# sephiroce/srf

Hardware: AMD Instinct MI355X
Metric: acoustic frames/sec through SRF (123-d fbank, 3-iter DR) at 1/2/4/8 MI355X (higher is better)
Workload: dtype fp32; 1 GPU; wsj_c4: SRF L=6 PH=CH=16 DIM=32 LPAD=RPAD=2 DR iter=3, train step (fwd+bwd+allreduce+Adam); utterances_per_gpu=28, frames_per_utterance=800, global_batch=28, parallelism=dp1, launch=hipgraph (fwd+CTC+bwd)

## Files before the change

include/srf.h:

```cpp
#ifndef SRF_H_
#define SRF_H_
#include <stddef.h>

#ifdef __cplusplus
extern "C" {
#endif

int srf_version(void);
const char* srf_last_error(void);

int srf_route_dr_auto_chunks(int B, int T, int N, int din, int lpad, int rpad, int J, int dout);
int srf_route_dr_split_table(int B, int T, int N, int din, int lpad, int rpad, int J, int dout, int n_chunks,
                             int* info, int* table, int capacity);
size_t srf_route_dr_saved_floats(int B, int T, int J, int dout, int iters);
size_t srf_route_dr_fwd_workspace(int B, int T, int N, int din, int lpad, int rpad, int J, int dout, int iters,
                                  int n_chunks);
size_t srf_route_dr_bwd_workspace(int B, int T, int N, int din, int lpad, int rpad, int J, int dout, int iters,
                                  int n_chunks);
int srf_route_dr_fwd(const float* emb, const float* W, const float* bias, int B, int T, int N, int din, int lpad,
                     int rpad, int J, int dout, int iters, int mask_first, int n_chunks, float* v_out,
                     float* saved, void* workspace, size_t workspace_bytes, void* stream);
size_t srf_route_dr_coupling_floats(int B, int T, int N, int din, int lpad, int rpad, int J, int dout, int iters);
int srf_route_dr_fwd_ex(const float* emb, const float* W, const float* bias, int B, int T, int N, int din, int lpad,
                        int rpad, int J, int dout, int iters, int mask_first, int n_chunks, float* v_out,
                        float* saved, float* couplings, void* workspace, size_t workspace_bytes, void* stream);
int srf_route_dr_bwd_ex(const float* emb, const float* W, const float* bias, int B, int T, int N, int din, int lpad,
                        int rpad, int J, int dout, int iters, int mask_first, int n_chunks, const float* saved,
                        const float* couplings, const float* g_v, float* g_emb, float* g_W, float* g_bias,
                        void* workspace, size_t workspace_bytes, void* stream);
int srf_route_dr_bwd_weights_ex(const float* emb, int B, int T, int N, int din, int lpad, int rpad, int J, int dout,
                                int iters, int mask_first, int n_chunks, const float* saved, const float* couplings,
                                float* g_W, float* g_bias, void* workspace, size_t workspace_bytes, void* stream);
int srf_route_dr_bwd_data_ex(const float* emb, const float* W, const float* bias, int B, int T, int N, int din,
                             int lpad, int rpad, int J, int dout, int iters, int mask_first, int n_chunks,
                             const float* saved, const float* couplings, const float* g_v, float* g_emb,
                             void* workspace, size_t workspace_bytes, void* stream);
int srf_set_seed_source(const void* step_counter);
int srf_set_fault_flag(void* flag);
int srf_route_dr_bwd(const float* emb, const float* W, const float* bias, int B, int T, int N, int din, int lpad,
                     int rpad, int J, int dout, int iters, int mask_first, int n_chunks, const float* saved,
                     const float* g_v, float* g_emb, float* g_W, float* g_bias, void* workspace,
                     size_t workspace_bytes, void* stream);
int srf_route_dr_bwd_data(const float* emb, const float* W, const float* bias, int B, int T, int N, int din,
                          int lpad, int rpad, int J, int dout, int iters, int mask_first, int n_chunks,
                          const float* saved, const float* g_v, float* g_emb, void* workspace,
                          size_t workspace_bytes, void* stream);
int srf_route_dr_bwd_weights(const float* emb, int B, int T, int N, int din, int lpad, int rpad, int J, int dout,
                             int iters, int mask_first, int n_chunks, float* g_W, float* g_bias, void* workspace,
                             size_t workspace_bytes, void* stream);

size_t srf_route_sdr_saved_floats(int B, int T, int J, int dout);
size_t srf_route_sdr_fwd_workspace(int B, int T, int N, int din, int lpad, int rpad, int J, int dout);
size_t srf_route_sdr_bwd_workspace(int B, int T, int N, int din, int lpad, int rpad, int J, int dout, int iters);
int srf_route_sdr_fwd(const float* emb, const float* W, const float* bias, int B, int T, int N, int din, int lpad,
                      int rpad, int J, int dout, int iters, int mask_first, float* v_out, float* saved,
                      void* workspace, size_t workspace_bytes, void* stream);
int srf_route_sdr_bwd(const float* emb, const float* W, const float* bias, int B, int T, int N, int din, int lpad,
                      int rpad, int J, int dout, int iters, int mask_first, const float* saved, const float* g_v,
                      float* g_emb, float* g_W, float* g_bias, void* workspace, size_t workspace_bytes,
                      void* stream);

#define SRF_SDR_MAX_ITEMS 8
typedef struct {
  int t0, t1;
  const float* emb;
  const float* W;
  const float* bias;
  const float* WT;
  float* u;
  int v0, vn;
  float* v;
  float* couplings;
  void* workspace;
  size_t workspace_bytes;
  const float* g_v;
// ... 204 lines not shown
```

srf_amd/_lib.py:

```python
import ctypes
import os

_HERE = os.path.dirname(os.path.abspath(__file__))
LIB_PATH = os.environ.get('SRF_LIB_PATH') or os.path.join(_HERE, 'libsrf.so')

_c_int, _c_size, _vp = ctypes.c_int, ctypes.c_size_t, ctypes.c_void_p

SDR_MAX_ITEMS = 8


class SdrRange(ctypes.Structure):
    _fields_ = [('t0', _c_int), ('t1', _c_int), ('emb', _vp), ('W', _vp), ('bias', _vp), ('WT', _vp),
                ('u', _vp), ('v0', _c_int), ('vn', _c_int), ('v', _vp), ('couplings', _vp),
                ('workspace', _vp), ('workspace_bytes', _c_size), ('g_v', _vp), ('carry', _vp),
                ('gu', _vp), ('g0', _c_int), ('gn', _c_int), ('g_emb', _vp), ('g_W', _vp), ('g_bias', _vp),
                ('accumulate', _c_int), ('u_bf16', _c_int), ('group', _c_int), ('gu_factored', _c_int)]


_ranges = ctypes.POINTER(SdrRange)

CAPSNORM_MAX_ITEMS = 8


class CapsnormRange(ctypes.Structure):
    _fields_ = [('t0', _c_int), ('t1', _c_int), ('layer', _c_int), ('x', _vp), ('gamma', _vp), ('beta', _vp),
                ('y', _vp), ('stat', _vp), ('g_y', _vp), ('g_x', _vp), ('gpart', _vp)]


_cn_ranges = ctypes.POINTER(CapsnormRange)

STREAM_ADVANCE_MAX = 32


class StreamBuf(ctypes.Structure):
    _fields_ = [('ptr', _vp), ('row_bytes', _c_size), ('rows_per_stream', _c_int), ('shift', _c_int),
                ('keep', _c_int)]

_SIGNATURES = {
    'srf_version': (_c_int, []),
    'srf_last_error': (ctypes.c_char_p, []),
    'srf_set_seed_source': (_c_int, [_vp]),
    'srf_set_fault_flag': (_c_int, [_vp]),
    'srf_route_dr_auto_chunks': (_c_int, [_c_int] * 8),
    'srf_route_dr_split_table': (_c_int, [_c_int] * 9 + [_vp, _vp, _c_int]),
    'srf_route_dr_saved_floats': (_c_size, [_c_int] * 5),
    'srf_route_dr_fwd_workspace': (_c_size, [_c_int] * 10),
    'srf_route_dr_bwd_workspace': (_c_size, [_c_int] * 10),
    'srf_route_dr_fwd': (_c_int, [_vp, _vp, _vp] + [_c_int] * 11 + [_vp, _vp, _vp, _c_size, _vp]),
    'srf_route_dr_bwd': (_c_int, [_vp, _vp, _vp] + [_c_int] * 11 + [_vp, _vp, _vp, _vp, _vp, _vp, _c_size, _vp]),
    'srf_route_dr_bwd_data': (_c_int, [_vp, _vp, _vp] + [_c_int] * 11 + [_vp, _vp, _vp, _vp, _c_size, _vp]),
    'srf_route_dr_bwd_weights': (_c_int, [_vp] + [_c_int] * 11 + [_vp, _vp, _vp, _c_size, _vp]),
    'srf_route_dr_coupling_floats': (_c_size, [_c_int] * 9),
    'srf_route_dr_fwd_ex': (_c_int, [_vp, _vp, _vp] + [_c_int] * 11 + [_vp, _vp, _vp, _vp, _c_size, _vp]),
    'srf_route_dr_bwd_ex': (_c_int, [_vp, _vp, _vp] + [_c_int] * 11 + [_vp] * 7 + [_c_size, _vp]),
    'srf_route_dr_bwd_data_ex': (_c_int, [_vp, _vp, _vp] + [_c_int] * 11 + [_vp] * 5 + [_c_size, _vp]),
    'srf_route_dr_bwd_weights_ex': (_c_int, [_vp] + [_c_int] * 11 + [_vp] * 5 + [_c_size, _vp]),
    'srf_route_sdr_saved_floats': (_c_size, [_c_int] * 4),
    'srf_route_sdr_fwd_workspace': (_c_size, [_c_int] * 8),
    'srf_route_sdr_bwd_workspace': (_c_size, [_c_int] * 9),
    'srf_route_sdr_fwd': (_c_int, [_vp, _vp, _vp] + [_c_int] * 10 + [_vp, _vp, _vp, _c_size, _vp]),
    'srf_route_sdr_bwd': (_c_int, [_vp, _vp, _vp] + [_c_int] * 10 + [_vp, _vp, _vp, _vp, _vp, _vp, _c_size, _vp]),
    'srf_route_sdr_pose': (_c_int, [_vp, _vp, _vp] + [_c_int] * 10 + [_vp, _c_int, _c_int, _vp]),
    'srf_route_sdr_pose_fp8': (_c_int, [_vp, _vp, _vp] + [_c_int] * 10 + [_vp, _c_int, _c_int, _vp]),
    'srf_route_sdr_recur_workspace': (_c_size, [_c_int] * 5),
    'srf_route_sdr_recur_zero_range': (_c_size, [_c_int] * 5 + [ctypes.POINTER(_c_size)]),
    'srf_route_sdr_coupling_floats': (_c_size, [_c_int] * 4),
    'srf_route_sdr_couplings_required': (_c_int, [_c_int] * 4),
    'srf_route_sdr_fact_floats': (_c_size, [_c_int] * 4),
    'srf_route_sdr_recur_fwd': (_c_int, [_vp] + [_c_int] * 11 + [_vp, _vp, _vp, _c_size, _vp]),
    'srf_route_sdr_recur_bwd': (_c_int, [_vp, _c_int, _c_int, _vp, _vp, _vp] + [_c_int] * 9
                                + [_vp, _vp, _c_int, _c_int, _vp, _c_size, _vp]),
    'srf_route_sdr_transpose_w': (_c_int, [_vp] + [_c_int] * 4 + [_vp, _vp]),
    'srf_route_sdr_gx': (_c_int, [_vp, _c_int, _c_int, _vp] + [_c_int] * 10 + [_vp, _vp]),
    'srf_route_sdr_gw': (_c_int, [_vp, _c_int, _c_int, _vp] + [_c_int] * 11 + [_vp, _vp, _vp]),
    'srf_route_sdr_pose_n': (_c_int, [_ranges] + [_c_int] * 10 + [_vp]),
    'srf_route_sdr_recur_fwd_n': (_c_int, [_ranges] + [_c_int] * 8 + [_vp]),
    'srf_route_sdr_recur_bwd_n': (_c_int, [_ranges] + [_c_int] * 8 + [_vp]),
    'srf_route_sdr_gx_n': (_c_int, [_ranges] + [_c_int] * 9 + [_vp]),
    'srf_route_sdr_gw_n': (_c_int, [_ranges] + [_c_int] * 9 + [_vp]),
    'srf_route_sdr_gx_gw_n': (_c_int, [_ranges] + [_c_int] * 9 + [_vp]),
    'srf_route_sdr_gx_gw_fact_n': (_c_int, [_ranges] + [_c_int] * 10 + [_vp]),
    'srf_cnnfe_out_dims': (_c_int, [_c_int, _c_int, ctypes.POINTER(_c_int), ctypes.POINTER(_c_int)]),
    'srf_cnnfe_saved_bytes': (_c_size, [_c_int] * 4),
    'srf_cnnfe_fwd_workspace': (_c_size, [_c_int] * 4),
    'srf_cnnfe_bwd_workspace': (_c_size, [_c_int] * 4),
    'srf_cnnfe_fwd': (_c_int, [_vp, _vp] + [_c_int] * 4 + [_vp] * 16 + [_c_int, ctypes.c_float, ctypes.c_ulonglong,
                                                                       _vp, _vp, _c_size, _vp, _c_size, _vp]),
    'srf_cnnfe_bwd': (_c_int, [_vp, _vp] + [_c_int] * 4 + [_vp] * 4 + [ctypes.c_float, ctypes.c_ulonglong]
                      + [_vp] * 15 + [_c_size, _vp]),
    'srf_cnnfe_bwd_parts': (_c_int, [_c_int, _vp, _vp] + [_c_int] * 4 + [_vp] * 4 + [ctypes.c_float, ctypes.c_ulonglong]
                            + [_vp] * 15 + [_c_size, _vp]),
    'srf_primary_caps_saved_bytes': (_c_size, [_c_int] * 4),
    'srf_primary_caps_bwd_workspace': (_c_size, [_c_int] * 5),
    'srf_primary_caps_fwd': (_c_int, [_vp, _vp] + [_c_int] * 5 + [_vp] * 8 + [_c_int, ctypes.c_float, ctypes.c_float,
                                                                           ctypes.c_ulonglong, _vp, _vp, _c_size, _vp]),
    'srf_primary_caps_bwd': (_c_int, [_vp, _vp] + [_c_int] * 5 + [_vp] * 5 + [_c_int, ctypes.c_float, ctypes.c_float,
                                                                           ctypes.c_ulonglong] + [_vp] * 12
                             + [_c_size, _vp]),
    'srf_primary_caps_fwd_ex': (_c_int, [_vp, _vp] + [_c_int] * 5 + [_vp] * 8
                                + [_c_int, ctypes.c_float, ctypes.c_float, ctypes.c_ulonglong, ctypes.c_float, _c_int,
                                   _vp, _vp, _c_size, _vp]),
    'srf_primary_caps_bwd_ex': (_c_int, [_vp, _vp] + [_c_int] * 5 + [_vp] * 5
                                + [_c_int, ctypes.c_float, ctypes.c_float, ctypes.c_ulonglong, ctypes.c_float]
                                + [_vp] * 12 + [_c_size, _vp]),
    'srf_capsnorm_bwd_workspace': (_c_size, [_c_int] * 3),
# ... 87 lines not shown
```

srf_amd/csrc/route_dr.hip:

```cpp
#include <algorithm>
#include <cmath>
#include <type_traits>

#include "srf_common.h"
#include "route_fwd32.h"
#include "../../include/srf.h"
#include "../../include/srf_prof.h"

namespace {

constexpr float kSquashEps = 1e-7f;

thread_local hipEvent_t* t_ev_start = nullptr;
thread_local hipEvent_t* t_ev_stop = nullptr;
thread_local int t_ev_n = 0;
constexpr int MODE_FWD = 0;
constexpr int MODE_BWD = 1;

using srf::DrGeom;

template <int KS>
__device__ __forceinline__ void load_vec(const float* __restrict__ p, float (&v)[KS]) {
  if constexpr (KS % 4 == 0) {
#pragma unroll
// ... 2356 lines not shown
  const bool bal = p.bal_G > 0;
  const int n_wg = bal ? p.bal_G : p.n_ftiles * p.n_chunks;
  info[0] = bal ? 1 : 0;
  info[1] = n_wg;
  info[2] = p.n_ftiles * in_n;
  info[3] = p.n_slots;
  info[4] = p.plan_arg;
  int n = 0;
  auto emit = [&](int w, int ft, int i0, int i1, int slot) {
    if (n < capacity) {
      int* row = table + (size_t)n * 5;
      row[0] = w, row[1] = ft, row[2] = i0, row[3] = i1, row[4] = slot;
    }
    ++n;
  };
  for (int w = 0; w < n_wg; ++w) {
    if (!bal) {
      const int ft = w / p.n_chunks, slot = w - ft * p.n_chunks;
      const int i0 = slot * p.chunk_len;
      emit(w, ft, std::min(i0, in_n), std::min(in_n, i0 + p.chunk_len), slot);
      continue;
    }
    int u = srf::bal_first(w, p.bal_U, p.bal_G);
    const int u1 = srf::bal_first(w + 1, p.bal_U, p.bal_G);
    while (u < u1) {
      const int ft = u / in_n, i0 = u - ft * in_n, i1 = std::min(in_n, i0 + (u1 - u));
      emit(w, ft, i0, i1, w - srf::bal_owner(ft * in_n, p.bal_U, p.bal_G));
      u += i1 - i0;
    }
  }
  return n;
}

size_t srf_route_dr_saved_floats(int B, int T, int J, int dout, int iters) {
  return (size_t)2 * iters * B * T * J * dout;
}

size_t srf_route_dr_fwd_workspace(int B, int T, int N, int din, int lpad, int rpad, int J, int dout, int iters,
                                  int n_chunks) {
  (void)iters;
  return query(B, T, N, din, lpad, rpad, J, dout, 1, n_chunks).fwd_bytes;
}

size_t srf_route_dr_bwd_workspace(int B, int T, int N, int din, int lpad, int rpad, int J, int dout, int iters,
                                  int n_chunks) {
  return query(B, T, N, din, lpad, rpad, J, dout, iters, n_chunks).ws.bytes;
}

size_t srf_route_dr_coupling_floats(int B, int T, int N, int din, int lpad, int rpad, int J, int dout, int iters) {
  const DrPlan p = query(B, T, N, din, lpad, rpad, J, dout, iters, 0);
  return p.can_store ? p.cpl.total : 0;
}

int srf_route_dr_fwd(const float* emb, const float* W, const float* bias, int B, int T, int N, int din, int lpad,
                     int rpad, int J, int dout, int iters, int mask_first, int n_chunks, float* v_out, float* saved,
                     void* workspace, size_t workspace_bytes, void* stream) {
  return srf_route_dr_fwd_ex(emb, W, bias, B, T, N, din, lpad, rpad, J, dout, iters, mask_first, n_chunks, v_out,
                             saved, nullptr, workspace, workspace_bytes, stream);
}

int srf_route_dr_fwd_ex(const float* emb, const float* W, const float* bias, int B, int T, int N, int din, int lpad,
                        int rpad, int J, int dout, int iters, int mask_first, int n_chunks, float* v_out,
                        float* saved, float* couplings, void* workspace, size_t workspace_bytes, void* stream) {
  DrPlan p;
  const int rc = enter(p, DrGeom{B, T, N, din, lpad, rpad, J, dout, iters, mask_first ? 1 : 0}, n_chunks,
                       emb && W && bias && v_out && saved && workspace, couplings != nullptr, true, workspace_bytes);
  if (rc) return rc;
  return dispatch_din(din, [&](auto D) {
    return fwd_impl<D>(p, emb, W, bias, v_out, saved, couplings, static_cast<float*>(workspace),
                       static_cast<hipStream_t>(stream));
  });
}

int srf_route_dr_bwd(const float* emb, const float* W, const float* bias, int B, int T, int N, int din, int lpad,
                     int rpad, int J, int dout, int iters, int mask_first, int n_chunks, const float* saved,
                     const float* g_v, float* g_emb, float* g_W, float* g_bias, void* workspace,
                     size_t workspace_bytes, void* stream) {
  return route_dr_bwd_entry(emb, W, bias, B, T, N, din, lpad, rpad, J, dout, iters, mask_first, n_chunks, saved,
                            nullptr, g_v, g_emb, g_W, g_bias, workspace, workspace_bytes, stream, true);
}

int srf_route_dr_bwd_ex(const float* emb, const float* W, const float* bias, int B, int T, int N, int din, int lpad,
                        int rpad, int J, int dout, int iters, int mask_first, int n_chunks, const float* saved,
                        const float* couplings, const float* g_v, float* g_emb, float* g_W, float* g_bias,
                        void* workspace, size_t workspace_bytes, void* stream) {
  return route_dr_bwd_entry(emb, W, bias, B, T, N, din, lpad, rpad, J, dout, iters, mask_first, n_chunks, saved,
                            couplings, g_v, g_emb, g_W, g_bias, workspace, workspace_bytes, stream, true);
}

int srf_route_dr_bwd_data(const float* emb, const float* W, const float* bias, int B, int T, int N, int din,
                          int lpad, int rpad, int J, int dout, int iters, int mask_first, int n_chunks,
                          const float* saved, const float* g_v, float* g_emb, void* workspace,
                          size_t workspace_bytes, void* stream) {
  return srf_route_dr_bwd_data_ex(emb, W, bias, B, T, N, din, lpad, rpad, J, dout, iters, mask_first, n_chunks, saved,
                                  nullptr, g_v, g_emb, workspace, workspace_bytes, stream);
}

int srf_route_dr_bwd_data_ex(const float* emb, const float* W, const float* bias, int B, int T, int N, int din,
                             int lpad, int rpad, int J, int dout, int iters, int mask_first, int n_chunks,
                             const float* saved, const float* couplings, const float* g_v, float* g_emb,
                             void* workspace, size_t workspace_bytes, void* stream) {
  float* unused = reinterpret_cast<float*>(workspace);
  return route_dr_bwd_entry(emb, W, bias, B, T, N, din, lpad, rpad, J, dout, iters, mask_first, n_chunks, saved,
                            couplings, g_v, g_emb, unused, unused, workspace, workspace_bytes, stream, false);
}

// ... 23 lines not shown
```

srf_amd/csrc/route_fwd32.hip:

```cpp
#include <cmath>
#include <cstdint>
#include <cstdlib>
#include <algorithm>
#include <type_traits>

#include "srf_common.h"
#include "route_fwd32.h"


#ifndef SRF_DR_IL
#define SRF_DR_IL 1
#endif

#ifndef SRF_DR_BAL_AUTO
#define SRF_DR_BAL_AUTO 1
#endif

namespace {

typedef __bf16 bf8 __attribute__((ext_vector_type(8)));
typedef __bf16 bf4 __attribute__((ext_vector_type(4)));
typedef _Float16 h8 __attribute__((ext_vector_type(8)));
typedef float f16v __attribute__((ext_vector_type(16)));

__device__ __forceinline__ f16v mfma32(const bf8& a, const bf8& b, const f16v& c) {
  return __builtin_amdgcn_mfma_f32_32x32x16_bf16(a, b, c, 0, 0, 0);
}
__device__ __forceinline__ f16v mfma32h(const h8& a, const h8& b, const f16v& c) {
  return __builtin_amdgcn_mfma_f32_32x32x16_f16(a, b, c, 0, 0, 0);
}

__device__ __forceinline__ float exp2i(int e) { return srf_exp2i(e); }
__device__ __forceinline__ int split_exp(float m) { return srf_split_exp(m); }

__device__ __forceinline__ void split3(float a, __bf16& a1, __bf16& a2, __bf16& a3) {
  a1 = (__bf16)a;
  const float r = a - (float)a1;
  a2 = (__bf16)r;
  a3 = (__bf16)(r - (float)a2);
}

__device__ __forceinline__ void split2h(float a, _Float16& a1, _Float16& a2) { srf_split2h(a, a1, a2); }

__device__ __forceinline__ void split8h(const float* __restrict__ src, bool ok, float s, _Float16* d1,
                                        _Float16* d2) {
  f4 lo = {0.f, 0.f, 0.f, 0.f}, hi = lo;
  if (ok) {
    lo = *reinterpret_cast<const f4*>(src);
    hi = *reinterpret_cast<const f4*>(src + 4);
  }
  const float v[8] = {lo.x, lo.y, lo.z, lo.w, hi.x, hi.y, hi.z, hi.w};
  h8 p1, p2;
#pragma unroll
  for (int k = 0; k < 8; ++k) {
    _Float16 a1, a2;
    split2h(v[k] * s, a1, a2);
    p1[k] = a1;
    p2[k] = a2;
  }
  *reinterpret_cast<h8*>(d1) = p1;
  *reinterpret_cast<h8*>(d2) = p2;
}

constexpr int kAbsBlocks = 128;
__global__ __launch_bounds__(256) void absmax_kernel(const float* __restrict__ a, size_t na,
                                                     const float* __restrict__ b, size_t nb, float* part) {
  const float* p = blockIdx.y ? b : a;
  const size_t n = blockIdx.y ? nb : na;
  float m = 0.f;
  const size_t stride = (size_t)gridDim.x * blockDim.x;
  size_t i = (size_t)blockIdx.x * blockDim.x + threadIdx.x;
  if ((reinterpret_cast<uintptr_t>(p) & 15) == 0) {
    const size_t n4 = n / 4;
    for (; i < n4; i += stride) {
      const f4 v = reinterpret_cast<const f4*>(p)[i];
      m = fmaxf(m, fmaxf(fmaxf(fabsf(v.x), fabsf(v.y)), fmaxf(fabsf(v.z), fabsf(v.w))));
    }
    i = n4 * 4 + (size_t)blockIdx.x * blockDim.x + threadIdx.x;
  }
  for (; i < n; i += stride) m = fmaxf(m, fabsf(p[i]));
#pragma unroll
  for (int o = 32; o >= 1; o >>= 1) m = fmaxf(m, __shfl_xor(m, o, 64));
  __shared__ float wm[4];
  if ((threadIdx.x & 63) == 0) wm[threadIdx.x >> 6] = m;
  __syncthreads();
  if (threadIdx.x == 0) part[blockIdx.y * kAbsBlocks + blockIdx.x] = fmaxf(fmaxf(wm[0], wm[1]), fmaxf(wm[2], wm[3]));
}

struct PrepArgs {
  const float *W, *bias, *emb;
  _Float16 *Ws, *xs;
  __bf16* bs;
  float *bsum, *WT, *xT;
  const float* part;
  float* hdr;
  int in_n, JD, JDp, din, n_chunks, chunk_len, F, N, T, lpad, Fp;
  int wt16;
  int xt16;
  size_t xplane;
  size_t n_a, n_b, n_c, n_d, n_e;
  size_t n_f, xt_block0;
};

constexpr int kXtTile = 64;

__global__ __launch_bounds__(256) void prep32_kernel(PrepArgs P) {
  if (P.n_f && blockIdx.x >= P.xt_block0) {
    __shared__ float tile[kXtTile][32 + 1];
    __shared__ int sbx;
    const int ntile = (P.Fp + kXtTile - 1) / kXtTile;
    const int blk = blockIdx.x - (int)P.xt_block0;
    const int i = blk / ntile, f0 = (blk - i * ntile) * kXtTile;
    const int w = i / P.N, n = i - w * P.N;
    if (P.xt16 && threadIdx.x < 64) {
      float m = 0.f;
      for (int k = threadIdx.x; k < kAbsBlocks; k += 64) m = fmaxf(m, P.part[kAbsBlocks + k]);
#pragma unroll
      for (int o = 32; o >= 1; o >>= 1) m = fmaxf(m, __shfl_xor(m, o, 64));
      if (threadIdx.x == 0) sbx = split_exp(m);
    }
    for (int k = threadIdx.x; k < kXtTile * P.din; k += blockDim.x) {
      const int fl = k / P.din, e = k - fl * P.din;
      const int f = f0 + fl;
      float v = 0.f;
      if (f < P.F) {
        const int b = f / P.T, t = f - b * P.T;
        const int ts = t + w - P.lpad;
        if (ts >= 0 && ts < P.T) v = P.emb[((size_t)(b * P.T + ts) * P.N + n) * P.din + e];
      }
      tile[fl][e] = v;
    }
    __syncthreads();
    if (P.xt16) {
      const float sc = exp2i(sbx);
      _Float16* x16 = reinterpret_cast<_Float16*>(P.xT);
      for (int k = threadIdx.x; k < (kXtTile / 16) * 32 * 2; k += blockDim.x) {
        const int hf = k & 1, e = (k >> 1) & 31, kb = k >> 6;
        const int fb = f0 + kb * 16;
        if (fb >= P.Fp) continue;
        h8 p1, p2;
#pragma unroll
        for (int q = 0; q < 8; ++q) {
          _Float16 a1, a2;
          split2h(tile[kb * 16 + hf * 8 + q][e] * sc, a1, a2);
          p1[q] = a1;
          p2[q] = a2;
        }
        const size_t base = (((size_t)i * (P.Fp / 16) + fb / 16) * 2 * 32 + e) * 16 + hf * 8;
        *reinterpret_cast<h8*>(x16 + base) = p1;
        *reinterpret_cast<h8*>(x16 + base + 32 * 16) = p2;
      }
      return;
    }
    for (int k = threadIdx.x; k < kXtTile * P.din; k += blockDim.x) {
      const int e = k / kXtTile, fl = k - e * kXtTile;
      const int f = f0 + fl;
      if (f < P.Fp) P.xT[((size_t)i * P.din + e) * P.Fp + f] = tile[fl][e];
    }
    return;
  }
  __shared__ int sexp[2];
  const size_t b0 = (size_t)blockIdx.x * blockDim.x, b1 = b0 + blockDim.x;
  const size_t ec = P.n_a + P.n_b, sd = ec + P.n_c, ed = sd + P.n_d;
  const bool split_work = b0 < ec || (b1 > sd && b0 < ed) || (P.wt16 && b1 > ed && b0 < ed + P.n_e);
  if (split_work && threadIdx.x < 128) {
    const int y = threadIdx.x >> 6, l = threadIdx.x & 63;
    float m = 0.f;
    for (int k = l; k < kAbsBlocks; k += 64) m = fmaxf(m, P.part[y * kAbsBlocks + k]);
#pragma unroll
    for (int o = 32; o >= 1; o >>= 1) m = fmaxf(m, __shfl_xor(m, o, 64));
    if (l == 0) sexp[y] = split_exp(m);
  }
  if (split_work) __syncthreads();
  const int aw = split_work ? sexp[0] : 0, bx = split_work ? sexp[1] : 0;
  if (blockIdx.x == 0 && threadIdx.x == 0) {
    P.hdr[0] = exp2i(-(aw + bx));
    P.hdr[1] = (float)aw;
    P.hdr[2] = (float)bx;
  }
  size_t idx = (size_t)blockIdx.x * blockDim.x + threadIdx.x;
  if (idx < P.n_a) {
    const size_t e0 = idx * 8;
    const int e = e0 % P.din;
    const size_t rr = e0 / P.din;
    const int row = rr % P.JDp;
    const size_t i = rr / P.JDp;
    const size_t nw = (size_t)P.in_n * P.JDp * P.din;
    split8h(P.W + (i * P.JD + min(row, P.JD - 1)) * P.din + e, row < P.JD, exp2i(aw), P.Ws + e0, P.Ws + nw + e0);
    return;
  }
  idx -= P.n_a;
  if (idx < P.n_b) {
    const int row = idx % P.JDp;
    const size_t i = idx / P.JDp;
    const float b = row < P.JD ? P.bias[i * P.JD + row] * exp2i(aw + bx) : 0.f;
    __bf16 b1, b2, b3;
    split3(b, b1, b2, b3);
    bf4 v = {b1, b2, b3, (__bf16)0.f};
    *reinterpret_cast<bf4*>(P.bs + idx * 4) = v;
    return;
  }
  idx -= P.n_b;
  if (idx < P.n_c) {
    const int c = idx / P.JD, row = idx - (size_t)c * P.JD;
    const int i0 = c * P.chunk_len, i1 = min(P.in_n, i0 + P.chunk_len);
    float acc = 0.f;
    for (int i = i0; i < i1; i += 8) {
      float v[8];
#pragma unroll
      for (int k = 0; k < 8; ++k) v[k] = i + k < i1 ? P.bias[(size_t)(i + k) * P.JD + row] : 0.f;
#pragma unroll
      for (int k = 0; k < 8; ++k) acc += v[k];
    }
    P.bsum[idx] = acc;
    return;
  }
  idx -= P.n_c;
  if (idx < P.n_d) {
    const size_t e0 = idx * 8;
    const size_t n_data = (size_t)P.F * P.N * P.din;
    const int e = e0 % P.din;
    const size_t rr = e0 / P.din;
    const int f = rr % P.F;
    const int n = rr / P.F;
    const bool ok = e0 < n_data;
    split8h(P.emb + ((size_t)(ok ? f : 0) * P.N + (ok ? n : 0)) * P.din + (ok ? e : 0), ok, exp2i(bx), P.xs + e0,
            P.xs + P.xplane + e0);
    return;
  }
  idx -= P.n_d;
  if (P.wt16 && idx < P.n_e) {
    const int e = idx % P.din;
    const size_t r1 = idx / P.din;
    const int h = r1 % 2;
    const size_t r2 = r1 / 2;
    const int nt16 = (P.JD + 15) / 16;
    const int t = r2 % nt16;
    const size_t i = r2 / nt16;
    const int row = t * 16 + 8 * h;
    const float* w = P.W + (i * P.JD + min(row, P.JD - 1)) * P.din + e;
    const float s = exp2i(aw);
    h8 p1, p2;
#pragma unroll
    for (int k = 0; k < 8; ++k) {
      _Float16 a1, a2;
      split2h(row + k < P.JD ? w[(size_t)k * P.din] * s : 0.f, a1, a2);
      p1[k] = a1;
      p2[k] = a2;
    }
    _Float16* d = reinterpret_cast<_Float16*>(P.WT);
    *reinterpret_cast<h8*>(d + idx * 8) = p1;
    *reinterpret_cast<h8*>(d + P.n_e * 8 + idx * 8) = p2;
    return;
  }
  if (idx < P.n_e) {
    const int e = idx % P.din;
    const size_t r1 = idx / P.din;
    const int g = r1 % 4;
    const size_t r2 = r1 / 4;
    const int nt16 = (P.JD + 15) / 16;
    const int t = r2 % nt16;
    const size_t i = r2 / nt16;
    const int row = t * 16 + 4 * g;
    const float* w = P.W + (i * P.JD + min(row, P.JD - 1)) * P.din + e;
    f4 v;
#pragma unroll
    for (int q = 0; q < 4; ++q) v[q] = row + q < P.JD ? w[(size_t)q * P.din] : 0.f;
// ... 1680 lines not shown
      best = c;
    }
  }
  p.n_chunks = best;
  p.chunk_len = (in_n + best - 1) / best;
  p.bal_G = 0;
  p.bal_U = 0;
  p.n_slots = best;
  p.plan_arg = best;
  {
    const long long U = (long long)n_ftiles * in_n;
    long long G = force_bal ? (n_chunks & (kBalFlag - 1)) : 0;
    if (G <= 0) G = slots;
    G = std::min(G, U);
    const bool fits = U * (G + 1) < (1ll << 31);
    if (fits && forced <= 0) {
      const int len = (int)((U + G - 1) / G);
      const int segs = (len - 1 + in_n - 1) / in_n + 1;
      int n_slots = 1;
      for (int ft = 0; ft < n_ftiles; ++ft) n_slots = std::max(n_slots, bal_tile_slots(ft, in_n, (int)U, (int)G));
      const double cost = (double)(len + kSegCost * segs) * (1.0 + 0.002 * n_slots);
      if (force_bal || (SRF_DR_BAL_AUTO && din == 32 && p.NW > 1 && p.TW == 2 && cost < best_cost)) {
        p.bal_G = (int)G;
        p.bal_U = (int)U;
        p.n_slots = n_slots;
        p.plan_arg = kBalFlag | (int)G;
      }
    }
  }
  p.ws_bsum = srf::align_up((size_t)best * JD * 4, 256);
  p.ws_slab = srf::align_up((size_t)std::max(best, p.n_slots) * F * JD * 4, 256);
  return p;
}

const float* fwd32_hdr(const Fwd32Shape& p, const void* planes) {
  return reinterpret_cast<const float*>(static_cast<const char*>(planes) + p.ws_w + p.ws_b + p.ws_x);
}
size_t fwd32_planes_bytes(const Fwd32Shape& p) { return p.ws_w + p.ws_b + p.ws_x + p.ws_h; }
size_t fwd32_scratch_bytes(const Fwd32Split& p) { return p.ws_bsum + p.ws_slab; }
size_t fwd32_workspace(const Fwd32Plan& p) { return fwd32_planes_bytes(p) + fwd32_scratch_bytes(p); }
float* fwd32_slab(const Fwd32Split& p, void* scratch) {
  return reinterpret_cast<float*>(static_cast<char*>(scratch) + p.ws_bsum);
}

size_t fwd32_lds(const Fwd32Shape& p) {
  return (size_t)p.NW * p.TW * 4 * 64 * 16 + (p.NW > 1 ? (size_t)2 * 32 * p.NW * 8 : 0);
}

int fwd32_prepare(const Fwd32Plan& p, const DrGeom& g, const float* emb, const float* W, const float* bias,
                  void* planes, void* scratch, float* WT, float* xT, hipStream_t st, bool wt16, bool xt16) {
  char* base = static_cast<char*>(planes);
  float* hdr = reinterpret_cast<float*>(base + p.ws_w + p.ws_b + p.ws_x);
  const int din = g.din;
  hipLaunchKernelGGL(absmax_kernel, dim3(kAbsBlocks, 2), dim3(256), 0, st, W, (size_t)g.in_n() * g.JD() * din, emb,
                     (size_t)g.F() * g.N * din, hdr + 64);
  SRF_LAUNCH_CHECK("absmax");
  PrepArgs P;
  P.W = W;
  P.bias = bias;
  P.emb = emb;
  P.Ws = reinterpret_cast<_Float16*>(base);
  P.bs = reinterpret_cast<__bf16*>(base + p.ws_w);
  P.xs = reinterpret_cast<_Float16*>(base + p.ws_w + p.ws_b);
  P.part = hdr + 64;
  P.hdr = hdr;
  P.bsum = reinterpret_cast<float*>(scratch);
  P.WT = WT;
  P.xT = xT;
  P.T = g.T;
  P.lpad = g.lpad;
  P.Fp = (g.F() + 15) / 16 * 16;
  P.in_n = g.in_n();
  P.JD = g.JD();
  P.JDp = p.JDp;
  P.din = din;
  P.n_chunks = p.n_chunks;
  P.chunk_len = p.chunk_len;
  P.F = g.F();
  P.N = g.N;
  P.xplane = p.xplane;
  P.n_a = (size_t)P.in_n * p.JDp * din / 8;
  P.n_b = (size_t)P.in_n * p.JDp;
  P.n_c = (size_t)p.n_chunks * P.JD;
  P.n_d = p.xplane / 8;
  SRF_REQUIRE(!wt16 || din == 32, "prep32: split W^T planes need din 32, got %d", din);
  P.wt16 = wt16 ? 1 : 0;
  SRF_REQUIRE(!xt16 || din == 32, "prep32: split x^T planes need din 32, got %d", din);
  P.xt16 = xt16 ? 1 : 0;
  P.n_e = WT ? (size_t)P.in_n * ((P.JD + 15) / 16) * (wt16 ? 2 : 4) * din : 0;
  SRF_REQUIRE(din <= 32, "prep32: xT tile holds din <= 32, got %d", din);
  P.n_f = xT ? (size_t)P.in_n * ((P.Fp + kXtTile - 1) / kXtTile) : 0;
  P.xt_block0 = (P.n_a + P.n_b + P.n_c + P.n_d + P.n_e + 255) / 256;
  hipLaunchKernelGGL(prep32_kernel, dim3(P.xt_block0 + P.n_f), dim3(256), 0, st, P);
  SRF_LAUNCH_CHECK("prep32");
  return SRF_OK;
}

template <int V>
using Int = std::integral_constant<int, V>;

template <class Fn>
static int dispatch_row(const DrGeom& g, const char* what, Fn&& fn) {
  if (g.din == g.dout) {
    switch (g.din) {
      case 8: return fn(Int<8>{}, Int<8>{});
      case 16: return fn(Int<16>{}, Int<16>{});
      case 32: return fn(Int<32>{}, Int<32>{});
    }
  }
  srf::set_error("%s: unsupported din %d dout %d", what, g.din, g.dout);
  return SRF_EUNSUPPORTED;
}

template <int DIN, class Fn>
static int dispatch_tiles(const Fwd32Shape& p, Fn&& fn) {
  if (p.TW == 2) {
    if constexpr (DIN <= 16) {
      return p.NW == 1 ? fn(Int<1>{}, Int<2>{}) : fn(Int<2>{}, Int<2>{});
    } else {
      switch (p.NW) {
        case 1: return fn(Int<1>{}, Int<2>{});
        case 2: return fn(Int<2>{}, Int<2>{});
        case 4: return fn(Int<4>{}, Int<2>{});
        default: return fn(Int<8>{}, Int<2>{});
      }
    }
  }
  switch (p.NW) {
    case 1: return fn(Int<1>{}, Int<kTW>{});
    case 2: return fn(Int<2>{}, Int<kTW>{});
    case 4: return fn(Int<4>{}, Int<kTW>{});
    default: return fn(Int<kMaxNW>{}, Int<kTW>{});
  }
}

template <int NW, int TW, class Kern, class... Args>
static int launch_rpass(const Fwd32Plan& p, const char* name, Kern piped, Kern plain, hipStream_t st,
                        const Args&... args) {
  const size_t lds = fwd32_lds(p);
  const Kern kern = (NW > 1 && TW <= 2) ? piped : plain;
  if (lds > 64 * 1024)
    SRF_HIP_TRY(hipFuncSetAttribute((const void*)kern, hipFuncAttributeMaxDynamicSharedMemorySize, (int)lds));
// ... 142 lines not shown
```

Baseline: 3.011 million frames/s.

## Add one-pass prep32 kernel that reads each input once via LDS tiles

```diff
diff --git a/include/srf.h b/include/srf.h
--- a/include/srf.h
+++ b/include/srf.h
@@ -21,6 +21,9 @@
                      int rpad, int J, int dout, int iters, int mask_first, int n_chunks, float* v_out,
                      float* saved, void* workspace, size_t workspace_bytes, void* stream);
 size_t srf_route_dr_coupling_floats(int B, int T, int N, int din, int lpad, int rpad, int J, int dout, int iters);
+#define SRF_DR_LAYOUT_N 17
+int srf_route_dr_operand_layout(int B, int T, int N, int din, int lpad, int rpad, int J, int dout, int iters,
+                                long long* out);
 int srf_route_dr_fwd_ex(const float* emb, const float* W, const float* bias, int B, int T, int N, int din, int lpad,
                         int rpad, int J, int dout, int iters, int mask_first, int n_chunks, float* v_out,
                         float* saved, float* couplings, void* workspace, size_t workspace_bytes, void* stream);
diff --git a/srf_amd/_lib.py b/srf_amd/_lib.py
--- a/srf_amd/_lib.py
+++ b/srf_amd/_lib.py
@@ -51,6 +51,7 @@
     'srf_route_dr_bwd_data': (_c_int, [_vp, _vp, _vp] + [_c_int] * 11 + [_vp, _vp, _vp, _vp, _c_size, _vp]),
     'srf_route_dr_bwd_weights': (_c_int, [_vp] + [_c_int] * 11 + [_vp, _vp, _vp, _c_size, _vp]),
     'srf_route_dr_coupling_floats': (_c_size, [_c_int] * 9),
+    'srf_route_dr_operand_layout': (_c_int, [_c_int] * 9 + [_vp]),
     'srf_route_dr_fwd_ex': (_c_int, [_vp, _vp, _vp] + [_c_int] * 11 + [_vp, _vp, _vp, _vp, _c_size, _vp]),
     'srf_route_dr_bwd_ex': (_c_int, [_vp, _vp, _vp] + [_c_int] * 11 + [_vp] * 7 + [_c_size, _vp]),
     'srf_route_dr_bwd_data_ex': (_c_int, [_vp, _vp, _vp] + [_c_int] * 11 + [_vp] * 5 + [_c_size, _vp]),
diff --git a/srf_amd/csrc/route_dr.hip b/srf_amd/csrc/route_dr.hip
--- a/srf_amd/csrc/route_dr.hip
+++ b/srf_amd/csrc/route_dr.hip
@@ -2432,6 +2432,41 @@
   return p.can_store ? p.cpl.total : 0;
 }
 
+int srf_route_dr_operand_layout(int B, int T, int N, int din, int lpad, int rpad, int J, int dout, int iters,
+                                long long* out) {
+  SRF_REQUIRE(out != nullptr, "operand_layout: null argument");
+  DrPlan p;
+  const DrGeom g{B, T, N, din, lpad, rpad, J, dout, iters, 0};
+  if (const int rc = check_geom(g)) return rc;
+  resolve(p, g, 0, true);
+  if (!p.couplings) {
+    srf::set_error("operand_layout: no coupling storage for this shape");
+    return SRF_EUNSUPPORTED;
+  }
+  const srf::Fwd32Shape& s = p.p32;
+  const size_t in_n = g.in_n(), Fp = padded_frames(g);
+  const size_t pl = p.cpl.planes;
+  const size_t v[SRF_DR_LAYOUT_N] = {pl,
+                                     2 * in_n * s.JDp * g.din * 2,
+                                     pl + s.ws_w / 4,
+                                     in_n * s.JDp * 8,
+                                     pl + (s.ws_w + s.ws_b) / 4,
+                                     2 * s.xplane * 2,
+                                     pl + (s.ws_w + s.ws_b + s.ws_x) / 4,
+                                     3 * sizeof(float),
+                                     p.cpl.WT,
+                                     in_n * g.din * ((size_t)g.NT() * 16) * 4,
+                                     p.cpl.xT,
+                                     in_n * g.din * Fp * 4,
+                                     (size_t)s.JDp,
+                                     s.xplane,
+                                     Fp,
+                                     p.gx == GxPass::kStored16 ? 1u : 0u,
+                                     p.gw == GwPass::kGw16s ? 1u : 0u};
+  for (int k = 0; k < SRF_DR_LAYOUT_N; ++k) out[k] = (long long)v[k];
+  return SRF_OK;
+}
+
 int srf_route_dr_fwd(const float* emb, const float* W, const float* bias, int B, int T, int N, int din, int lpad,
                      int rpad, int J, int dout, int iters, int mask_first, int n_chunks, float* v_out, float* saved,
                      void* workspace, size_t workspace_bytes, void* stream) {
diff --git a/srf_amd/csrc/route_fwd32.hip b/srf_amd/csrc/route_fwd32.hip
--- a/srf_amd/csrc/route_fwd32.hip
+++ b/srf_amd/csrc/route_fwd32.hip
@@ -14,6 +14,10 @@
 
 #ifndef SRF_DR_BAL_AUTO
 #define SRF_DR_BAL_AUTO 1
+#endif
+
+#ifndef SRF_PREP32_ONEPASS
+#define SRF_PREP32_ONEPASS 1
 #endif
 
 namespace {
@@ -63,8 +67,12 @@
 }
 
 constexpr int kAbsBlocks = 128;
-__global__ __launch_bounds__(256) void absmax_kernel(const float* __restrict__ a, size_t na,
-                                                     const float* __restrict__ b, size_t nb, float* part) {
+constexpr int kAbsThreads = SRF_PREP32_ONEPASS ? 1024 : 256;
+__device__ __forceinline__ float absmax4(const f4& v) {
+  return fmaxf(fmaxf(fabsf(v.x), fabsf(v.y)), fmaxf(fabsf(v.z), fabsf(v.w)));
+}
+__global__ __launch_bounds__(kAbsThreads) void absmax_kernel(const float* __restrict__ a, size_t na,
+                                                             const float* __restrict__ b, size_t nb, float* part) {
   const float* p = blockIdx.y ? b : a;
   const size_t n = blockIdx.y ? nb : na;
   float m = 0.f;
@@ -72,6 +80,13 @@
   size_t i = (size_t)blockIdx.x * blockDim.x + threadIdx.x;
   if ((reinterpret_cast<uintptr_t>(p) & 15) == 0) {
     const size_t n4 = n / 4;
+    if (SRF_PREP32_ONEPASS) {
+      for (; i + 3 * stride < n4; i += 4 * stride) {
+        const f4* q = reinterpret_cast<const f4*>(p) + i;
+        const f4 v0 = q[0], v1 = q[stride], v2 = q[2 * stride], v3 = q[3 * stride];
+        m = fmaxf(m, fmaxf(fmaxf(absmax4(v0), absmax4(v1)), fmaxf(absmax4(v2), absmax4(v3))));
+      }
+    }
     for (; i < n4; i += stride) {
       const f4 v = reinterpret_cast<const f4*>(p)[i];
       m = fmaxf(m, fmaxf(fmaxf(fabsf(v.x), fabsf(v.y)), fmaxf(fabsf(v.z), fabsf(v.w))));
@@ -81,10 +96,14 @@
   for (; i < n; i += stride) m = fmaxf(m, fabsf(p[i]));
 #pragma unroll
   for (int o = 32; o >= 1; o >>= 1) m = fmaxf(m, __shfl_xor(m, o, 64));
-  __shared__ float wm[4];
+  __shared__ float wm[kAbsThreads / 64];
   if ((threadIdx.x & 63) == 0) wm[threadIdx.x >> 6] = m;
   __syncthreads();
-  if (threadIdx.x == 0) part[blockIdx.y * kAbsBlocks + blockIdx.x] = fmaxf(fmaxf(wm[0], wm[1]), fmaxf(wm[2], wm[3]));
+  if (threadIdx.x == 0) {
+#pragma unroll
+    for (int k = 1; k < kAbsThreads / 64; ++k) m = fmaxf(m, wm[k]);
+    part[blockIdx.y * kAbsBlocks + blockIdx.x] = m;
+  }
 }
 
 struct PrepArgs {
@@ -100,9 +119,206 @@
   size_t xplane;
   size_t n_a, n_b, n_c, n_d, n_e;
   size_t n_f, xt_block0;
+  int rpad, n_xblk, n_wblk, w_bpc;
 };
 
 constexpr int kXtTile = 64;
+
+__device__ __forceinline__ void prep_bs(const PrepArgs& P, size_t idx, int aw, int bx) {
+  const int row = idx % P.JDp;
+  const size_t i = idx / P.JDp;
+  const float b = row < P.JD ? P.bias[i * P.JD + row] * exp2i(aw + bx) : 0.f;
+  __bf16 b1, b2, b3;
+  split3(b, b1, b2, b3);
+  bf4 v = {b1, b2, b3, (__bf16)0.f};
+  *reinterpret_cast<bf4*>(P.bs + idx * 4) = v;
+}
+
+__device__ __forceinline__ void prep_bsum(const PrepArgs& P, size_t idx) {
+  const int c = idx / P.JD, row = idx - (size_t)c * P.JD;
+  const int i0 = c * P.chunk_len, i1 = min(P.in_n, i0 + P.chunk_len);
+  float acc = 0.f;
+  for (int i = i0; i < i1; i += 8) {
+    float v[8];
+#pragma unroll
+    for (int k = 0; k < 8; ++k) v[k] = i + k < i1 ? P.bias[(size_t)(i + k) * P.JD + row] : 0.f;
+#pragma unroll
+    for (int k = 0; k < 8; ++k) acc += v[k];
+  }
+  P.bsum[idx] = acc;
+}
+
+constexpr int kXHaloMax = 16;
+constexpr int kXImgStride = kXtTile + kXHaloMax + 1;
+
+__device__ __forceinline__ int wave_split_exp(const float* __restrict__ part, int y) {
+  const int l = threadIdx.x & 63;
+  float m = fmaxf(part[y * kAbsBlocks + l], part[y * kAbsBlocks + 64 + l]);
+  static_assert(kAbsBlocks == 128, "two block maxima per lane");
+#pragma unroll
+  for (int o = 32; o >= 1; o >>= 1) m = fmaxf(m, __shfl_xor(m, o, 64));
+  return split_exp(m);
+}
+
+__device__ __forceinline__ void split4w(const f4& v, float s, uint32_t (&w)[4]) {
+#pragma unroll
+  for (int j = 0; j < 4; ++j) {
+    _Float16 a1, a2;
+    split2h(v[j] * s, a1, a2);
+    w[j] = (uint32_t)__builtin_bit_cast(uint16_t, a1) | ((uint32_t)__builtin_bit_cast(uint16_t, a2) << 16);
+  }
+}
+__device__ __forceinline__ uint32_t pack_hi(uint32_t a, uint32_t b) { return (a & 0xffffu) | (b << 16); }
+__device__ __forceinline__ uint32_t pack_lo(uint32_t a, uint32_t b) { return (a >> 16) | (b & 0xffff0000u); }
+
+typedef uint32_t u2v __attribute__((ext_vector_type(2)));
+typedef uint32_t u4v __attribute__((ext_vector_type(4)));
+
+constexpr int kWTileStride = 36;
+constexpr int kPrepLdsWords = 4 * 64 * kWTileStride;
+static_assert(32 * kXImgStride + kXtTile <= kPrepLdsWords && (32 * kXImgStride) % 4 == 0, "x image + tt fit");
+
+__device__ __forceinline__ void prep_x_tile(const PrepArgs& P, int blk, uint32_t* lds) {
+  uint32_t* const img = lds;
+  int* const tt = reinterpret_cast<int*>(lds + 32 * kXImgStride);
+  const int tid = threadIdx.x;
+  const int tile = blk / P.N, n = blk - tile * P.N;
+  const int f0 = tile * kXtTile;
+  const int nrow = kXtTile + P.lpad + P.rpad;
+  constexpr int kIt = (kXtTile + kXHaloMax) * 8 / 256 + ((kXtTile + kXHaloMax) * 8 % 256 ? 1 : 0);
+  f4 v[kIt];
+#pragma unroll
+  for (int it = 0; it < kIt; ++it) {
+    const int k = tid + it * 256, r = k >> 3, e4 = k & 7;
+    const int fr = f0 - P.lpad + r;
+    v[it] = f4{0.f, 0.f, 0.f, 0.f};
+    if (r < nrow && fr >= 0 && fr < P.F)
+      v[it] = *reinterpret_cast<const f4*>(P.emb + ((size_t)fr * P.N + n) * 32 + 4 * e4);
+  }
+  if (tid < kXtTile) {
+    const int f = f0 + tid;
+    tt[tid] = f < P.F ? f - (f / P.T) * P.T : -(1 << 24);
+  }
+  if (blk == 0 && tid < 8) {
+    const h8 z = {};
+    *reinterpret_cast<h8*>(P.xs + (size_t)(tid >> 2) * P.xplane + (P.xplane - 32) + (tid & 3) * 8) = z;
+  }
+  const float sc = exp2i(wave_split_exp(P.part, 1));
+#pragma unroll
+  for (int it = 0; it < kIt; ++it) {
+    const int k = tid + it * 256, r = k >> 3, e4 = k & 7;
+    const int fr = f0 - P.lpad + r;
+    if (r >= nrow) continue;
+    uint32_t w[4];
+    split4w(v[it], sc, w);
+    if (P.xT) {
+#pragma unroll
+      for (int j = 0; j < 4; ++j) img[(4 * e4 + j) * kXImgStride + r] = w[j];
+    }
+    if (r >= P.lpad && r < P.lpad + kXtTile && fr < P.F) {
+      _Float16* d = P.xs + ((size_t)n * P.F + fr) * 32 + 4 * e4;
+      *reinterpret_cast<u2v*>(d) = u2v{pack_hi(w[0], w[1]), pack_hi(w[2], w[3])};
+      *reinterpret_cast<u2v*>(d + P.xplane) = u2v{pack_lo(w[0], w[1]), pack_lo(w[2], w[3])};
+    }
+  }
+  if (!P.xT) return;
+  __syncthreads();
+  const int e = tid & 31, hf = (tid >> 5) & 1, kb = tid >> 6;
+  const int fb = f0 + kb * 16;
+  if (fb >= P.Fp) return;
+  int t8[8];
+  {
+    const u4v a = *reinterpret_cast<const u4v*>(&tt[kb * 16 + hf * 8]);
+    const u4v b = *reinterpret_cast<const u4v*>(&tt[kb * 16 + hf * 8 + 4]);
+#pragma unroll
+    for (int q = 0; q < 4; ++q) t8[q] = (int)a[q] - P.lpad, t8[4 + q] = (int)b[q] - P.lpad;
+  }
+  _Float16* x16 = reinterpret_cast<_Float16*>(P.xT);
+  const uint32_t* col = img + e * kXImgStride + kb * 16 + hf * 8;
+  const int nwin = P.lpad + P.rpad + 1;
+  for (int w = 0; w < nwin; ++w) {
+    uint32_t c[8];
+#pragma unroll
+    for (int q = 0; q < 8; ++q) c[q] = (uint32_t)(t8[q] + w) < (uint32_t)P.T ? col[w + q] : 0u;
+    const size_t i = (size_t)w * P.N + n;
+    const size_t base = ((i * (P.Fp / 16) + fb / 16) * 2 * 32 + e) * 16 + hf * 8;
+    *reinterpret_cast<u4v*>(x16 + base) =
+        u4v{pack_hi(c[0], c[1]), pack_hi(c[2], c[3]), pack_hi(c[4], c[5]), pack_hi(c[6], c[7])};
+    *reinterpret_cast<u4v*>(x16 + base + 32 * 16) =
+        u4v{pack_lo(c[0], c[1]), pack_lo(c[2], c[3]), pack_lo(c[4], c[5]), pack_lo(c[6], c[7])};
+  }
+}
+
+__device__ __forceinline__ void prep_w_rows(const PrepArgs& P, int blk, uint32_t* lds) {
+  const int i = blk / P.w_bpc, rb = blk - i * P.w_bpc;
+  const int lane = threadIdx.x & 63, wv = threadIdx.x >> 6;
+  const int e4 = lane & 7, g = lane >> 3;
+  const int rw0 = rb * 256 + wv * 64;
+  const bool active = rw0 < P.JDp;
+  uint32_t* const t = lds + wv * 64 * kWTileStride;
+  f4 v[8];
+#pragma unroll
+  for (int k = 0; k < 8; ++k) {
+    const int row = rw0 + g * 8 + k;
+    v[k] = f4{0.f, 0.f, 0.f, 0.f};
+    if (row < P.JD) v[k] = *reinterpret_cast<const f4*>(P.W + ((size_t)i * P.JD + row) * 32 + 4 * e4);
+  }
+  const float s = exp2i(wave_split_exp(P.part, 0));
+#pragma unroll
+  for (int k = 0; k < 8; ++k) {
+    uint32_t w[4];
+    split4w(v[k], s, w);
+    *reinterpret_cast<u4v*>(t + (g * 8 + k) * kWTileStride + 4 * e4) = u4v{w[0], w[1], w[2], w[3]};
+  }
+  __syncthreads();
+  if (!active) return;
+  const size_t nw = (size_t)P.in_n * P.JDp * 32;
+#pragma unroll
+  for (int it = 0; it < 4; ++it) {
+    const int rl = it * 16 + (lane >> 2), c8 = (lane & 3) * 8;
+    const u4v a = *reinterpret_cast<const u4v*>(t + rl * kWTileStride + c8);
+    const u4v b = *reinterpret_cast<const u4v*>(t + rl * kWTileStride + c8 + 4);
+    _Float16* d = P.Ws + ((size_t)i * P.JDp + rw0 + rl) * 32 + c8;
+    *reinterpret_cast<u4v*>(d) = u4v{pack_hi(a[0], a[1]), pack_hi(a[2], a[3]), pack_hi(b[0], b[1]), pack_hi(b[2], b[3])};
+    *reinterpret_cast<u4v*>(d + nw) =
+        u4v{pack_lo(a[0], a[1]), pack_lo(a[2], a[3]), pack_lo(b[0], b[1]), pack_lo(b[2], b[3])};
+  }
+  if (P.WT == nullptr) return;
+  const int nt16 = (P.JD + 15) / 16;
+  const int e = lane & 31;
+#pragma unroll
+  for (int it = 0; it < 4; ++it) {
+    const int g2 = it * 2 + (lane >> 5);
+    const int r0 = rw0 + g2 * 8;
+    if (r0 >= nt16 * 16) continue;
+    uint32_t c[8];
+#pragma unroll
+    for (int q = 0; q < 8; ++q) c[q] = t[(g2 * 8 + q) * kWTileStride + e];
+    _Float16* d = reinterpret_cast<_Float16*>(P.WT) + (((size_t)i * nt16 * 2 + r0 / 8) * 32 + e) * 8;
+    *reinterpret_cast<u4v*>(d) = u4v{pack_hi(c[0], c[1]), pack_hi(c[2], c[3]), pack_hi(c[4], c[5]), pack_hi(c[6], c[7])};
+    *reinterpret_cast<u4v*>(d + P.n_e * 8) =
+        u4v{pack_lo(c[0], c[1]), pack_lo(c[2], c[3]), pack_lo(c[4], c[5]), pack_lo(c[6], c[7])};
+  }
+}
+
+__global__ __launch_bounds__(256) void prep32_onepass_kernel(PrepArgs P) {
+  __shared__ __attribute__((aligned(16))) uint32_t lds[kPrepLdsWords];
+  int blk = blockIdx.x;
+  if (blk < P.n_xblk) return prep_x_tile(P, blk, lds);
+  blk -= P.n_xblk;
+  if (blk < P.n_wblk) return prep_w_rows(P, blk, lds);
+  blk -= P.n_wblk;
+  const int aw = wave_split_exp(P.part, 0), bx = wave_split_exp(P.part, 1);
+  if (blk == 0 && threadIdx.x == 0) {
+    P.hdr[0] = exp2i(-(aw + bx));
+    P.hdr[1] = (float)aw;
+    P.hdr[2] = (float)bx;
+  }
+  size_t idx = (size_t)blk * blockDim.x + threadIdx.x;
+  if (idx < P.n_b) return prep_bs(P, idx, aw, bx);
+  idx -= P.n_b;
+  if (idx < P.n_c) prep_bsum(P, idx);
+}
 
 __global__ __launch_bounds__(256) void prep32_kernel(PrepArgs P) {
   if (P.n_f && blockIdx.x >= P.xt_block0) {
@@ -191,28 +407,12 @@
   }
   idx -= P.n_a;
   if (idx < P.n_b) {
-    const int row = idx % P.JDp;
-    const size_t i = idx / P.JDp;
-    const float b = row < P.JD ? P.bias[i * P.JD + row] * exp2i(aw + bx) : 0.f;
-    __bf16 b1, b2, b3;
-    split3(b, b1, b2, b3);
-    bf4 v = {b1, b2, b3, (__bf16)0.f};
-    *reinterpret_cast<bf4*>(P.bs + idx * 4) = v;
+    prep_bs(P, idx, aw, bx);
     return;
   }
   idx -= P.n_b;
   if (idx < P.n_c) {
-    const int c = idx / P.JD, row = idx - (size_t)c * P.JD;
-    const int i0 = c * P.chunk_len, i1 = min(P.in_n, i0 + P.chunk_len);
-    float acc = 0.f;
-    for (int i = i0; i < i1; i += 8) {
-      float v[8];
-#pragma unroll
-      for (int k = 0; k < 8; ++k) v[k] = i + k < i1 ? P.bias[(size_t)(i + k) * P.JD + row] : 0.f;
-#pragma unroll
-      for (int k = 0; k < 8; ++k) acc += v[k];
-    }
-    P.bsum[idx] = acc;
+    prep_bsum(P, idx);
     return;
   }
   idx -= P.n_c;
@@ -1999,8 +2199,8 @@
   char* base = static_cast<char*>(planes);
   float* hdr = reinterpret_cast<float*>(base + p.ws_w + p.ws_b + p.ws_x);
   const int din = g.din;
-  hipLaunchKernelGGL(absmax_kernel, dim3(kAbsBlocks, 2), dim3(256), 0, st, W, (size_t)g.in_n() * g.JD() * din, emb,
-                     (size_t)g.F() * g.N * din, hdr + 64);
+  hipLaunchKernelGGL(absmax_kernel, dim3(kAbsBlocks, 2), dim3(kAbsThreads), 0, st, W,
+                     (size_t)g.in_n() * g.JD() * din, emb, (size_t)g.F() * g.N * din, hdr + 64);
   SRF_LAUNCH_CHECK("absmax");
   PrepArgs P;
   P.W = W;
@@ -2035,6 +2235,22 @@
   SRF_REQUIRE(!xt16 || din == 32, "prep32: split x^T planes need din 32, got %d", din);
   P.xt16 = xt16 ? 1 : 0;
   P.n_e = WT ? (size_t)P.in_n * ((P.JD + 15) / 16) * (wt16 ? 2 : 4) * din : 0;
+  P.rpad = g.rpad;
+  P.n_xblk = P.n_wblk = P.w_bpc = 0;
+  P.n_f = P.xt_block0 = 0;
+  if (SRF_PREP32_ONEPASS && din == 32 && (!WT || wt16) && (!xT || xt16) && P.JD % 8 == 0 &&
+      g.lpad + g.rpad <= kXHaloMax) {
+    const size_t n_xblk = (size_t)((P.F + kXtTile - 1) / kXtTile) * P.N;
+    P.w_bpc = (P.JDp + 255) / 256;
+    const size_t n_wblk = (size_t)P.in_n * P.w_bpc;
+    const size_t n_blk = n_xblk + n_wblk + (P.n_b + P.n_c + 255) / 256;
+    SRF_REQUIRE(n_blk < (1ull << 31), "prep32: %zu blocks", n_blk);
+    P.n_xblk = (int)n_xblk;
+    P.n_wblk = (int)n_wblk;
+    hipLaunchKernelGGL(prep32_onepass_kernel, dim3((unsigned)n_blk), dim3(256), 0, st, P);
+    SRF_LAUNCH_CHECK("prep32_onepass");
+    return SRF_OK;
+  }
   SRF_REQUIRE(din <= 32, "prep32: xT tile holds din <= 32, got %d", din);
   P.n_f = xT ? (size_t)P.in_n * ((P.Fp + kXtTile - 1) / kXtTile) : 0;
   P.xt_block0 = (P.n_a + P.n_b + P.n_c + P.n_d + P.n_e + 255) / 256;
```

Result: faster. 3.065 million frames/s, median of 6 (+1.8%).
